# ruizhecao96/CMGAN

Measured on AMD Instinct MI355X. Metric: enhanced audio frames/sec (16 kHz, 2 s clips, batch 32 per GPU), higher is better.
Workload: dtype f32 storage/accumulate; products as 3 x f16 split MFMA (fp32-class accuracy); 1 GPU; configs[1]: batch=32 x 2 s synthetic 16 kHz noisy clips per GPU, n_fft=400 hop=100, TSCNet(64,201) random-init, full pipeline wav->wav; mfma_mode=f16x3, launch=hipGraph replay, batch_per_gpu=32, global_batch=32, frames_per_clip=321, parallelism=dp1

## Files before the change

### cmgan_amd/csrc/attn32_x3.hip

```cpp
#if defined(X3_SINGLE) && defined(A32_STAMP)
#undef A32_STAMP
#endif
#include "kernels.h"
#include <string.h>
#include <stdlib.h>

namespace X3_NS {

typedef float f32x16 __attribute__((ext_vector_type(16)));

__device__ __forceinline__ f32x16 mfma3216(f16x8 a, f16x8 b, f32x16 c) {
    return __builtin_amdgcn_mfma_f32_32x32x16_f16(a, b, c, 0, 0, 0);
}
__device__ __forceinline__ f32x16 mfma3216l(f16x8 a, f16x8 b, f32x16 c) {
    return X3_TERMS == 3 ? __builtin_amdgcn_mfma_f32_32x32x16_f16(a, b, c, 0, 0, 0) : c;
}
__device__ __forceinline__ f32x16 zero16() {
    f32x16 z;
#pragma unroll
    for (int i = 0; i < 16; ++i) z[i] = 0.f;
    return z;
}
#ifdef A32_STAMP
#define A32_SLOTS 2048
__device__ unsigned long long g_a32_stamp[A32_SLOTS][64];
struct A32Stamp {
    unsigned long long t, acc[16];
    int chunks;
};
#define A32_STAMP_ARG , A32Stamp& sp
#define A32_STAMP_PASS , sp
#define A32_STAMP_PTR , A32Stamp* spp
#define A32_STAMP_PTRPASS , &sp
#define A32_MARK(ph)                                            \
    do {                                                        \
        __builtin_amdgcn_sched_barrier(0);                      \
        const unsigned long long _t = __builtin_readcyclecounter(); \
        sp.acc[ph] += _t - sp.t;                                \
        sp.t = _t;                                              \
        __builtin_amdgcn_sched_barrier(0);                      \
    } while (0)
#else
#define A32_STAMP_ARG
#define A32_STAMP_PASS
#define A32_STAMP_PTR
#define A32_STAMP_PTRPASS
#define A32_MARK(ph) do { } while (0)
#endif

__device__ __forceinline__ float red_h_max(float v) {
    float b;
    const float a = xchg32(v, b);
    return fmaxf(a, b);
}
__device__ __forceinline__ float red_h_sum(float v) {
    float b;
    const float a = xchg32(v, b);
    return a + b;
}

#ifndef XCD_ORDER
#define XCD_ORDER 1
#endif
#define XNTB 2
#define XWAVES 8

__device__ __forceinline__ void ln_split32(const f32x4 (&x)[4], f16x8 (&bh)[2], f16x8 (&bl)[2]) {
    float mean, rstd;
    ln_stats(x, mean, rstd);
    f32x4 xh[4];
#pragma unroll
    for (int kb = 0; kb < 4; ++kb) xh[kb] = (x[kb] - splat4(mean)) * splat4(rstd);
    split8(xh[0], xh[1], bh[0], bl[0]);
    split8(xh[2], xh[3], bh[1], bl[1]);
}

__global__ __launch_bounds__(512) void qkv32_x3_kernel(const float* __restrict__ x, TokMap m, int Lt,
                                                       const _Float16* __restrict__ wi, const float* __restrict__ b,
                                                       _Float16* __restrict__ qimg, _Float16* __restrict__ kimg,
                                                       _Float16* __restrict__ vimg, int ntiles) {
    __shared__ __attribute__((aligned(16))) _Float16 wlds[24576];
    __shared__ float scratch[XWAVES * 32 * 17];
    __shared__ __attribute__((aligned(16))) float bias_l[192];
    stage_lds16<3072, 512>(wi, wlds);
    for (int i = threadIdx.x; i < 192; i += blockDim.x) bias_l[i] = b[i];
    __syncthreads();
    const int lane = threadIdx.x & 63, c = lane & 15, g = lane >> 4, wv = threadIdx.x >> 6;
    const int row32 = lane & 31, hh = lane >> 5;
    float* T = scratch + wv * (32 * 17);

#pragma unroll 1
    for (int tile = blockIdx.x * XWAVES + wv; tile < ntiles; tile += gridDim.x * XWAVES) {
        const int n = tile / Lt, it = tile - n * Lt;
        f16x8 xbh[XNTB][2], xbl[XNTB][2];
#pragma unroll
        for (int tb = 0; tb < XNTB; ++tb) {
            int l = it * 32 + tb * 16 + c;
            if (l >= m.L) l = m.L - 1;
            const long row = (long)(n / m.inner) * m.outer + (long)(n % m.inner) * m.istride + (long)l * m.lstride;
            f32x4 xr[4];
#pragma unroll
            for (int kb = 0; kb < 4; ++kb) xr[kb] = ldg4(x + row * 64 + 16 * kb + 4 * g);
            ln_split32(xr, xbh[tb], xbl[tb]);
        }
#pragma unroll 2
        for (int ob = 0; ob < 12; ++ob) {
            const f32x4 bias = *reinterpret_cast<const f32x4*>(&bias_l[16 * ob + 4 * g]);
            f32x4 acc[XNTB];
#pragma unroll
            for (int tb = 0; tb < XNTB; ++tb) acc[tb] = bias;
            lin_acc_x3<2, XNTB>(wlds + ob * 2048 + lane * 8, xbh, xbl, acc);
            const int which = ob >> 2, h = ob & 3;
            const long nh = (long)n * 4 + h;
            if (which < 2) {
                _Float16* img = (which == 0 ? qimg : kimg) + (nh * Lt + it) * 1024;
#pragma unroll
                for (int tb = 0; tb < XNTB; ++tb) {
                    f16x4 hi, lo;
                    split4(acc[tb], hi, lo);
                    _Float16* p = img + ((g >> 1) * 32 + 16 * tb + c) * 8 + 4 * (g & 1);
                    *reinterpret_cast<f16x4*>(p) = hi;
                    *reinterpret_cast<f16x4*>(p + 512) = lo;
                }
            } else {
                wave_lds_fence();
#pragma unroll
                for (int tb = 0; tb < XNTB; ++tb)
#pragma unroll
                    for (int r = 0; r < 4; ++r) T[(16 * tb + c) * 17 + 4 * g + r] = acc[tb][r];
                wave_lds_fence();
#pragma unroll
                for (int grp = 0; grp < 2; ++grp) {
                    f32x4 va, vb;
#pragma unroll
                    for (int r = 0; r < 4; ++r) {
                        va[r] = T[(16 * grp + 4 * hh + r) * 17 + (row32 & 15)];
                        vb[r] = T[(16 * grp + 8 + 4 * hh + r) * 17 + (row32 & 15)];
                    }
                    f16x8 vh, vl;
                    split8(va, vb, vh, vl);
                    const f16x8 out = row32 < 16 ? vh : vl;
                    *reinterpret_cast<f16x8*>(vimg + ((nh * Lt + it) * 2 + grp) * 512 + lane * 8) = out;
                }
            }
        }
    }
}

#ifndef A32_OCC
#define A32_OCC 2
#endif
#ifndef A32_RSEQ
#define A32_RSEQ 1
#endif
#define A32_HI 12.0f
#define A32_LO -4.0f
#define A32_RFL (96 * 32)

struct A32State {
    float m, run, l;
};

typedef unsigned u32x4v __attribute__((ext_vector_type(4)));
__device__ __forceinline__ __amdgpu_buffer_rsrc_t a32_rsrc(const void* base, unsigned bytes) {
    return __builtin_amdgcn_make_buffer_rsrc(const_cast<void*>(base), 0, bytes, 0x00020000);
}
__device__ __forceinline__ f16x8 buf_h8(__amdgpu_buffer_rsrc_t r, unsigned voff, unsigned soff) {
    return __builtin_bit_cast(f16x8, __builtin_amdgcn_raw_buffer_load_b128(r, voff, soff, 0));
}

struct A32Ctx {
    __amdgpu_buffer_rsrc_t qr, kr, vr, er;
    unsigned lane16, eoff, eplane2;
    float* R;
    int wbase, rbase;
    int Lt, L, max_pos, i0, a, hh;
    const unsigned char* mk;
    const char* xbase;
    const char* bo;
};

__device__ __forceinline__ void a32_load_e(const A32Ctx& c, int i0, int n, int t, f16x8& eh, f16x8& el) {
    int row = c.max_pos - (i0 - 64 * n + 32 - 32 * t) + c.a;
#ifdef A32_FAKEE
    row = c.max_pos - 32 + 32 * t + c.a;
#endif
    row = row < 0 ? 0 : (row > 2 * c.max_pos ? 2 * c.max_pos : row);
    const unsigned off = (unsigned)row * 16u + c.eoff;
    eh = buf_h8(c.er, off, 0);
    el = buf_h8(c.er, off, c.eplane2);
}
__device__ __forceinline__ void a32_load_k(const A32Ctx& c, int n, int jt, f16x8& kh, f16x8& kl) {
    int kt = 2 * n + jt;
    kt = kt < c.Lt ? kt : c.Lt - 1;
#ifdef A32_FAKEKV
    kt = jt;
#endif
    kh = buf_h8(c.kr, c.lane16, (unsigned)kt * 2048u);
    kl = buf_h8(c.kr, c.lane16 + 1024u, (unsigned)kt * 2048u);
}
__device__ __forceinline__ f16x8 a32_load_v(const A32Ctx& c, int n, int grp4) {
    int gr = 4 * n + grp4;
    gr = gr < 2 * c.Lt ? gr : 2 * c.Lt - 1;
#ifdef A32_FAKEKV
    gr = grp4 & 1;
#endif
    return buf_h8(c.vr, c.lane16, (unsigned)gr * 1024u);
}

template <int NKT, bool FULL, bool MASK>
__device__ __forceinline__ void a32_softmax(f32x16 (&s)[2], const A32Ctx& c, int j0, A32State& st, f32x16& o,
                                            bool qvalid A32_STAMP_PTR) {
    float mx = -INFINITY;
#pragma unroll
    for (int jt = 0; jt < NKT; ++jt) {
#pragma unroll
        for (int v = 0; v < 16; ++v) {
            float xv = s[jt][v] - st.m;
            const int key = j0 + 32 * jt + 8 * (v >> 2) + 4 * c.hh + (v & 3);
            if (!FULL) xv = key < c.L ? xv : -INFINITY;
            if (MASK && (FULL || key < c.L)) xv = qvalid ? (c.mk[key] ? xv : -INFINITY) : 0.f;
            s[jt][v] = xv;
            mx = fmaxf(mx, xv);
        }
    }
    const float run = fmaxf(st.run, red_h_max(mx));
#ifdef A32_STAMP
    if (spp) { A32Stamp& sp = *spp; A32_MARK(11); }
#endif
    const bool dead = MASK && run == -INFINITY;
    const bool drift = !dead && (run > A32_HI || run < A32_LO);
    float runk = run;
    if (__any(drift)) {
        const float shift = dead ? 0.f : run;
        const float alpha = st.l > 0.f ? __builtin_amdgcn_exp2f(-shift) : 1.0f;
#pragma unroll
        for (int jt = 0; jt < NKT; ++jt)
#pragma unroll
            for (int v = 0; v < 16; ++v) s[jt][v] -= shift;
        st.l *= alpha;
#pragma unroll
        for (int v = 0; v < 16; ++v) o[v] *= alpha;
        st.m += shift;
        if (!dead) runk = 0.f;
    }
    st.run = runk;
    float psum = 0.f;
#pragma unroll
    for (int jt = 0; jt < NKT; ++jt)
#pragma unroll
        for (int v = 0; v < 16; ++v) {
            const float p = __builtin_amdgcn_exp2f(s[jt][v]);
            s[jt][v] = p;
            psum += p;
        }
    st.l += psum;
}

template <int NKT, bool FULL, bool LAST, bool MASK>
__device__ __forceinline__ void a32_chunk(const A32Ctx& c, int n, int i0n, int nn, f16x8& qh, f16x8& ql, f16x8 (&eh)[3], f16x8 (&el)[3],
                                          f16x8 (&kh)[2], f16x8 (&kl)[2], f16x8 (&va)[4], A32State& st, f32x16& o,
                                          bool qvalid, const unsigned (&xo)[2], f32x4 (&xold)[2], f32x4& bias
                                          A32_STAMP_ARG) {
    constexpr int NT = NKT + 1;
#ifndef A32_NO_R
#pragma unroll
    for (int t = 0; t < NT; ++t) {
        f32x16 r = mfma3216(eh[t], qh, zero16());
        if (t == 0) A32_MARK(8);
        r = mfma3216l(eh[t], ql, r);
        r = mfma3216l(el[t], qh, r);
#pragma unroll
        for (int v = 0; v < 16; ++v) c.R[c.wbase + (32 * t + 8 * (v >> 2) + (v & 3)) * 32] = r[v];
        if (A32_RSEQ && (t & 1)) __builtin_amdgcn_sched_barrier(0);
    }
#ifndef A32_NO_LD
#pragma unroll
    for (int t = 0; t < 3; ++t) a32_load_e(c, i0n, nn, t, eh[t], el[t]);
#endif
#endif
    A32_MARK(1);
    wave_lds_fence();
    f32x16 s[2];
#ifndef A32_NO_R
#pragma unroll
    for (int jt = 0; jt < NKT; ++jt) {
#pragma unroll
        for (int v = 0; v < 16; ++v) s[jt][v] = c.R[c.rbase + (32 * jt + 8 * (v >> 2) + (v & 3)) * 32];
    }
#else
    s[0] = zero16(); s[1] = zero16();
#endif
    wave_lds_fence();
    A32_MARK(9);
#pragma unroll
    for (int jt = 0; jt < NKT; ++jt) {
        s[jt] = mfma3216(kh[jt], qh, s[jt]);
        s[jt] = mfma3216l(kh[jt], ql, s[jt]);
        s[jt] = mfma3216l(kl[jt], qh, s[jt]);
    }
#ifndef A32_NO_LD
#pragma unroll
    for (int jt = 0; jt < 2; ++jt) a32_load_k(c, nn, jt, kh[jt], kl[jt]);
    if (LAST) {
        const int itn = (i0n >> 5) < c.Lt ? (i0n >> 5) : c.Lt - 1;
        qh = buf_h8(c.qr, c.lane16, (unsigned)itn * 2048u);
        ql = buf_h8(c.qr, c.lane16 + 1024u, (unsigned)itn * 2048u);
    }
#endif
    A32_MARK(2);
#ifndef A32_NO_SM
    a32_softmax<NKT, FULL, MASK>(s, c, 64 * n, st, o, qvalid A32_STAMP_PTRPASS);
#else
    st.l += s[0][0] + s[1][5];
#endif
    A32_MARK(3);
    if (LAST) {
#pragma unroll
        for (int i = 0; i < 2; ++i) xold[i] = *reinterpret_cast<const f32x4*>(c.xbase + xo[i]);
        bias = *reinterpret_cast<const f32x4*>(c.bo + (c.lane16 >> 8) * 16u);
    }
#ifdef A32_NO_PV
#pragma unroll
    for (int v = 0; v < 16; ++v) o[v] += s[0][v] + s[1][v];
#else
#pragma unroll
    for (int jt = 0; jt < NKT; ++jt) {
#pragma unroll
        for (int half = 0; half < 2; ++half) {
            f32x4 pa, pb;
#pragma unroll
            for (int r = 0; r < 4; ++r) {
                pa[r] = s[jt][8 * half + r];
                pb[r] = s[jt][8 * half + 4 + r];
            }
            f16x8 ph, pl;
            split8(pa, pb, ph, pl);
            o = mfma3216(va[2 * jt + half], ph, o);
            if (jt == 0 && half == 0) A32_MARK(10);
            o = mfma3216l(va[2 * jt + half], pl, o);
        }
    }
#endif
#ifndef A32_NO_LD
#pragma unroll
    for (int g4 = 0; g4 < 4; ++g4) va[g4] = a32_load_v(c, nn, g4);
#endif
    A32_MARK(4);
#ifdef A32_STAMP
    ++sp.chunks;
#endif
}

#ifndef A32_TPB
#define A32_TPB 4
#endif
#ifndef A32_TPB_SHORT
#define A32_TPB_SHORT 16
#endif
#ifndef A32_SLOTS_PER_GPU
#define A32_SLOTS_PER_GPU 512
#endif
#ifndef A32_PERSIST_LONG
#define A32_PERSIST_LONG 0
#endif
#ifndef A32_GROUP
#define A32_GROUP 64
#endif
template <bool MASK>
__global__ __launch_bounds__(256, MASK ? 1 : A32_OCC) void attn32_out_x3_kernel(const _Float16* __restrict__ qimg,
                                                                     const _Float16* __restrict__ kimg,
                                                                     const _Float16* __restrict__ vimg,
                                                                     const _Float16* __restrict__ eimg, int max_pos,
                                                                     float* __restrict__ x, TokMap m,
                                                                     const _Float16* __restrict__ woi,
                                                                     const float* __restrict__ bo, int Lt, int tpb,
                                                                     int bps, long nblocks,
                                                                     const unsigned char* __restrict__ mask) {
    __shared__ __attribute__((aligned(16))) float rbuf[4][A32_RFL];
    __shared__ __attribute__((aligned(16))) f32x4 stash[2][4][2][64];
    __shared__ __attribute__((aligned(16))) _Float16 wo_l[8192];
#ifdef A32_LONE
    __shared__ float lone_pad[8192];
    if (max_pos < 0) lone_pad[threadIdx.x] = 1.f;
#endif
#ifdef A32_STAMP
    A32Stamp sp;
    sp.t = __builtin_readcyclecounter();
    sp.chunks = 0;
#pragma unroll
    for (int i = 0; i < 16; ++i) sp.acc[i] = 0;
#endif
    const int lane = threadIdx.x & 63, wv = __builtin_amdgcn_readfirstlane(threadIdx.x >> 6);
    const long lblk = XCD_ORDER ? (long)(blockIdx.x & 7) * (gridDim.x >> 3) + (blockIdx.x >> 3) : (long)blockIdx.x;
    if (lblk >= nblocks) return;
    stage_lds16<1024, 256>(woi, wo_l);
    const int n = __builtin_amdgcn_readfirstlane((int)((unsigned)lblk / (unsigned)bps));
    const int it0 = ((int)lblk - n * bps) * tpb, it1 = it0 + tpb < Lt ? it0 + tpb : Lt;
    const long nh = (long)n * 4 + wv;
    const int L = m.L;
    A32Ctx c;
    c.a = lane & 31; c.hh = lane >> 5;
    c.R = rbuf[wv];
    c.wbase = 4 * c.hh * 32 + c.a;
    c.rbase = (32 + 4 * c.hh - c.a) * 32 + c.a;
    c.Lt = Lt; c.L = L; c.max_pos = max_pos;
    c.kr = a32_rsrc(kimg + nh * Lt * 1024, (unsigned)Lt * 2048u);
    c.vr = a32_rsrc(vimg + nh * Lt * 1024, (unsigned)Lt * 2048u);
    c.er = a32_rsrc(eimg, (unsigned)(2 * max_pos + 1) * 64u);
    c.qr = a32_rsrc(qimg + nh * Lt * 1024, (unsigned)Lt * 2048u);
    c.lane16 = (unsigned)lane * 16u;
    c.eoff = (unsigned)c.hh * (unsigned)(2 * max_pos + 1) * 16u;
    c.eplane2 = (unsigned)(2 * max_pos + 1) * 32u;
    c.mk = MASK ? mask + (long)n * L : nullptr;
    const int c16 = lane & 15, g16 = lane >> 4;
    const int nq = __builtin_amdgcn_readfirstlane(n / m.inner);
    char* xbase = reinterpret_cast<char*>(x + ((long)nq * m.outer + (long)(n - nq * m.inner) * m.istride) * 64 + 16 * wv);
    const unsigned xstride = (unsigned)m.lstride * 256u, xlane = (unsigned)g16 * 16u;

    c.xbase = xbase;
    c.bo = reinterpret_cast<const char*>(bo + 16 * wv);
    f16x8 qh = buf_h8(c.qr, c.lane16, (unsigned)it0 * 2048u), ql = buf_h8(c.qr, c.lane16 + 1024u, (unsigned)it0 * 2048u);
    f16x8 eh[3], el[3], kh[2], kl[2], va[4];
#pragma unroll
    for (int t = 0; t < 3; ++t) a32_load_e(c, 32 * it0, 0, t, eh[t], el[t]);
#pragma unroll
    for (int jt = 0; jt < 2; ++jt) a32_load_k(c, 0, jt, kh[jt], kl[jt]);
#pragma unroll
    for (int g4 = 0; g4 < 4; ++g4) va[g4] = a32_load_v(c, 0, g4);
    const int nfull = L >> 6, tail = L & 63;
    A32_MARK(0);

#pragma unroll 1
    for (int it = it0; it < it1; ++it) {
        c.i0 = 32 * it;
        bool qvalid = true;
        if (MASK) {
            const int lq = c.i0 + c.a;
            qvalid = c.mk[lq < L ? lq : L - 1] != 0;
        }
        A32State st;
        st.m = 0.f; st.run = -INFINITY; st.l = 0.f;
        f32x16 o = zero16();
        const int i0x = c.i0 + 32;
        unsigned xo[2];
        f32x4 xold[2], bias;
#pragma unroll
        for (int i = 0; i < 2; ++i) {
            const int l = c.i0 + 16 * i + c16;
            xo[i] = (unsigned)(l < L ? l : L - 1) * xstride + xlane;
        }
#define A32_ARGS qh, ql, eh, el, kh, kl, va, st, o, qvalid, xo, xold, bias A32_STAMP_PASS
        if (tail) {
#pragma unroll 1
            for (int ch = 0; ch < nfull; ++ch) a32_chunk<2, true, false, MASK>(c, ch, c.i0, ch + 1, A32_ARGS);
            if (tail > 32) a32_chunk<2, false, true, MASK>(c, nfull, i0x, 0, A32_ARGS);
            else a32_chunk<1, false, true, MASK>(c, nfull, i0x, 0, A32_ARGS);
        } else {
#pragma unroll 1
            for (int ch = 0; ch + 1 < nfull; ++ch) a32_chunk<2, true, false, MASK>(c, ch, c.i0, ch + 1, A32_ARGS);
            a32_chunk<2, true, true, MASK>(c, nfull - 1, i0x, 0, A32_ARGS);
        }
#undef A32_ARGS
        const float inv = __builtin_amdgcn_rcpf(red_h_sum(st.l));
        f32x4 oa, ob;
#pragma unroll
        for (int r = 0; r < 4; ++r) {
            oa[r] = (o[r] + o[8 + r]) * inv;
            ob[r] = (o[4 + r] + o[12 + r]) * inv;
        }
#ifdef A32_NO_EPI
        if (c.i0 + c16 < L) *reinterpret_cast<f32x4*>(xbase + xo[0]) = oa + ob + xold[0] + xold[1] + bias;
        continue;
#endif
        const int par = (it - it0) & 1;
        const _Float16* wp = wo_l + wv * 2048 + lane * 8;
        stash[par][wv][c.a >> 4][c.hh * 16 + (c.a & 15)] = oa;
        stash[par][wv][c.a >> 4][(2 + c.hh) * 16 + (c.a & 15)] = ob;
        A32_MARK(5);
#ifndef A32_NO_BAR
        __syncthreads();
#endif
        A32_MARK(6);
        const f16x8 ah0 = *reinterpret_cast<const f16x8*>(wp), al0 = *reinterpret_cast<const f16x8*>(wp + 512);
        const f16x8 ah1 = *reinterpret_cast<const f16x8*>(wp + 1024), al1 = *reinterpret_cast<const f16x8*>(wp + 1536);
#pragma unroll
        for (int i = 0; i < 2; ++i) {
            f16x8 bh0, bl0, bh1, bl1;
            split8(stash[par][0][i][lane], stash[par][1][i][lane], bh0, bl0);
            split8(stash[par][2][i][lane], stash[par][3][i][lane], bh1, bl1);
            f32x4 acc = bias;
            acc = mfma32h(ah0, bh0, acc);
            acc = mfma32l(ah0, bl0, acc);
            acc = mfma32l(al0, bh0, acc);
            acc = mfma32h(ah1, bh1, acc);
            acc = mfma32l(ah1, bl1, acc);
            acc = mfma32l(al1, bh1, acc);
            if (c.i0 + 16 * i + c16 < L) *reinterpret_cast<f32x4*>(xbase + xo[i]) = xold[i] + acc;
        }
        A32_MARK(7);
    }
#ifdef A32_STAMP
    if (lane == 0) {
        const int b = L < 200 ? 32 : 0;
        unsigned long long* slot = g_a32_stamp[(blockIdx.x * 4 + (threadIdx.x >> 6)) & (A32_SLOTS - 1)];
#pragma unroll
        for (int i = 0; i < 16; ++i) atomicAdd(&slot[b + i], sp.acc[i]);
        atomicAdd(&slot[b + 16], 1ull);
        atomicAdd(&slot[b + 17], (unsigned long long)sp.chunks);
    }
#endif
}

#ifdef A32_STAMP
extern "C" int cmgan_dbg_a32_stamps(unsigned long long* out, int reset) {
    hipDeviceSynchronize();
    static unsigned long long host[A32_SLOTS][64];
    hipError_t e = hipMemcpyFromSymbol(host, HIP_SYMBOL(g_a32_stamp), sizeof host);
    for (int i = 0; i < 64; ++i) {
        out[i] = 0;
        for (int sl = 0; sl < A32_SLOTS; ++sl) out[i] += host[sl][i];
    }
    if (e == hipSuccess && reset) {
        memset(host, 0, sizeof host);
        e = hipMemcpyToSymbol(HIP_SYMBOL(g_a32_stamp), host, sizeof host);
    }
    return e == hipSuccess ? 0 : -1;
}
#endif

#ifndef ASP_OCC
#define ASP_OCC 2
#endif
#define ASP_P 100
#define ASP_RFL (32 * ASP_P)
#define ASP_SB() __builtin_amdgcn_sched_barrier(0)
#if defined(A32_STAMP) && (A32_STAMP + 0 == 2)
#define ASP_FMARK(ph) do { } while (0)
#define ASP_CMARK(ph) A32_MARK(ph)
#else
#define ASP_FMARK(ph) A32_MARK(ph)
#define ASP_CMARK(ph) do { } while (0)
#endif
#ifndef ASP_ABL
#define ASP_ABL 0
#endif

__device__ __forceinline__ f32x16 splat16(float v) {
    f32x16 z;
#pragma unroll
    for (int i = 0; i < 16; ++i) z[i] = v;
    return z;
}

struct AspCtx {
    __amdgpu_buffer_rsrc_t qr, kr, vr, er;
    unsigned lane16, evoff, eplane2;
    float* Rw;
    const float* Rr;
    int Lt, L, max_pos, a, hh, lpad;
};

template <bool CLAMP>
__device__ __forceinline__ void asp_load_e(const AspCtx& c, int i0, int n, int t, f16x8& eh, f16x8& el) {
    if (CLAMP) {
        int row = c.max_pos - (i0 - 64 * n + 32 - 32 * t) + c.a;
        row = row < 0 ? 0 : (row > 2 * c.max_pos ? 2 * c.max_pos : row);
        const unsigned off = (unsigned)row * 16u + c.evoff;
        eh = buf_h8(c.er, off, 0);
        el = buf_h8(c.er, off, c.eplane2);
    } else {
        i0 = i0 < c.lpad ? i0 : c.lpad;
        const unsigned so = (unsigned)(64 * n + 32 * t - i0 + c.lpad) * 16u;
        eh = buf_h8(c.er, c.evoff, so);
        el = buf_h8(c.er, c.evoff, so + c.eplane2);
    }
}
__device__ __forceinline__ void asp_load_k(const AspCtx& c, unsigned so, int n, int jt, f16x8& kh, f16x8& kl) {
    int kt = 2 * n + jt;
    kt = kt < c.Lt ? kt : c.Lt - 1;
    kh = buf_h8(c.kr, c.lane16, so + (unsigned)kt * 2048u);
    kl = buf_h8(c.kr, c.lane16 + 1024u, so + (unsigned)kt * 2048u);
}
__device__ __forceinline__ f16x8 asp_load_v(const AspCtx& c, unsigned so, int n, int grp4) {
    int gr = 4 * n + grp4;
    gr = gr < 2 * c.Lt ? gr : 2 * c.Lt - 1;
    return buf_h8(c.vr, c.lane16, so + (unsigned)gr * 1024u);
}
__device__ __forceinline__ void asp_load_q(const AspCtx& c, unsigned so, int it, f16x8& qh, f16x8& ql) {
    it = it < c.Lt ? it : c.Lt - 1;
    qh = buf_h8(c.qr, c.lane16, so + (unsigned)it * 2048u);
    ql = buf_h8(c.qr, c.lane16 + 1024u, so + (unsigned)it * 2048u);
}
struct AspTile {
    unsigned so;
    int it;
};

__device__ __forceinline__ f32x16 asp_eq(const f16x8& eh, const f16x8& el, const f16x8& qh, const f16x8& ql,
                                         const f32x16& negm) {
    f32x16 r = mfma3216(eh, qh, negm);
    r = mfma3216l(eh, ql, r);
    return mfma3216l(el, qh, r);
}
__device__ __forceinline__ void asp_wwrite(const AspCtx& c, int t, const f32x16& r) {
#pragma unroll
    for (int k = 0; k < 4; ++k) {
        f32x4 w = {r[4 * k], r[4 * k + 1], r[4 * k + 2], r[4 * k + 3]};
        *reinterpret_cast<f32x4*>(c.Rw + 32 * t + 8 * k) = w;
    }
}
template <int NKT>
__device__ __forceinline__ void asp_wread(const AspCtx& c, f32x16 (&sn)[2]) {
#pragma unroll
    for (int jt = 0; jt < NKT; ++jt)
#pragma unroll
        for (int v = 0; v < 16; ++v) sn[jt][v] = c.Rr[32 * jt + 8 * (v >> 2) + (v & 3)];
}
__host__ __device__ constexpr int asp_koff(int jt, int v) { return 32 * jt + 8 * (v >> 2) + (v & 3); }
template <int TAILK = 0>
__device__ __forceinline__ void asp_exp8(const f32x16 (&s)[2], int g, float& psum, f16x8& ph, f16x8& pl) {
    if (ASP_ABL == 3) {
        f32x4 a = {s[g >> 1][8 * (g & 1)], s[g >> 1][8 * (g & 1) + 1], s[g >> 1][8 * (g & 1) + 2], s[g >> 1][8 * (g & 1) + 3]};
        f32x4 b = {s[g >> 1][8 * (g & 1) + 4], s[g >> 1][8 * (g & 1) + 5], s[g >> 1][8 * (g & 1) + 6], s[g >> 1][8 * (g & 1) + 7]};
        ph = __builtin_bit_cast(f16x8, a); pl = __builtin_bit_cast(f16x8, b);
        psum += a[0];
        return;
    }
    f32x4 pa, pb;
#pragma unroll
    for (int r = 0; r < 4; ++r) {
        const bool la = TAILK == 0 || asp_koff(g >> 1, 8 * (g & 1) + r) < TAILK;
        const bool lb = TAILK == 0 || asp_koff(g >> 1, 8 * (g & 1) + 4 + r) < TAILK;
        pa[r] = la ? __builtin_amdgcn_exp2f(s[g >> 1][8 * (g & 1) + r]) : 0.f;
        pb[r] = lb ? __builtin_amdgcn_exp2f(s[g >> 1][8 * (g & 1) + 4 + r]) : 0.f;
        if (la) psum += pa[r];
        if (lb) psum += pb[r];
    }
    asm volatile("" : "+v"(psum));
    split8(pa, pb, ph, pl);
}
__host__ __device__ constexpr int asp_live_groups(int TAILK, int NKT) { return TAILK > 0 ? (TAILK + 15) / 16 : 2 * NKT; }
__device__ __forceinline__ void asp_pv(f32x16& o, const f16x8& va, const f16x8& ph, const f16x8& pl) {
    if (ASP_ABL == 4 || ASP_ABL == 10) {
        o[0] += (float)ph[0] + (float)pl[0] + (float)va[0];
        return;
    }
    o = mfma3216(va, ph, o);
    o = mfma3216l(va, pl, o);
}

template <int NKT, bool CLAMP, bool LASTQ>
__device__ __forceinline__ void asp_front(const AspCtx& c, AspTile tn, int nn, f16x8& qh, f16x8& ql,
                                          f16x8 (&eh)[3], f16x8 (&el)[3], f16x8 (&kh)[2], f16x8 (&kl)[2],
                                          const f32x16& negm, f32x16 (&sn)[2]) {
#pragma unroll
    for (int t = 0; t <= NKT; ++t) {
        const f32x16 r = asp_eq(eh[t], el[t], qh, ql, negm);
        asp_wwrite(c, t, r);
        ASP_SB();
    }
    if (!LASTQ) { eh[0] = eh[2]; el[0] = el[2]; }
#pragma unroll
    for (int t = LASTQ ? 0 : 1; t < 3; ++t) asp_load_e<CLAMP>(c, 32 * tn.it, nn, t, eh[t], el[t]);
    wave_lds_fence();
    asp_wread<NKT>(c, sn);
    wave_lds_fence();
#pragma unroll
    for (int jt = 0; jt < NKT; ++jt) sn[jt] = asp_eq(kh[jt], kl[jt], qh, ql, sn[jt]);
    if (LASTQ) asp_load_q(c, tn.so, tn.it, qh, ql);
#pragma unroll
    for (int jt = 0; jt < 2; ++jt) asp_load_k(c, tn.so, nn, jt, kh[jt], kl[jt]);
    if (LASTQ) __builtin_amdgcn_s_waitcnt(0x0f70);
}

template <int NKT, int TAILK = 0>
__device__ __forceinline__ void asp_back(f32x16 (&s)[2], A32State& st, f32x16& o, const f16x8 (&va)[4]) {
    float psum = 0.f;
#pragma unroll
    for (int g = 0; g < asp_live_groups(TAILK, NKT); ++g) {
        f16x8 ph, pl;
        asp_exp8<TAILK>(s, g, psum, ph, pl);
        asp_pv(o, va[g], ph, pl);
    }
    st.l += psum;
}

template <int NKT, bool FULL, int TAILK = 0>
__device__ __forceinline__ float asp_max(const AspCtx& c, f32x16 (&s)[2], int j0) {
    float mx[2] = {-INFINITY, -INFINITY};
#pragma unroll
    for (int jt = 0; jt < NKT; ++jt)
#pragma unroll
        for (int v = 0; v < 16; ++v) {
            if (!FULL && TAILK > 0) {
                const int koff = asp_koff(jt, v);
                if (koff >= TAILK) { s[jt][v] = -INFINITY; continue; }
                if (koff + 4 >= TAILK) s[jt][v] = c.hh ? -INFINITY : s[jt][v];
            } else if (!FULL) {
                const int key = j0 + 32 * jt + 8 * (v >> 2) + 4 * c.hh + (v & 3);
                s[jt][v] = key < c.L ? s[jt][v] : -INFINITY;
            }
            mx[jt] = fmaxf(mx[jt], s[jt][v]);
        }
    return red_h_max(fmaxf(mx[0], mx[1]));
}

template <int NKT, bool FULL, int TAILK = 0>
__device__ __forceinline__ void asp_reference(const AspCtx& c, f32x16 (&s)[2], int j0, A32State& st, f32x16& o,
                                              f32x16& negm) {
    const float run = fmaxf(st.run, asp_max<NKT, FULL, TAILK>(c, s, j0));
    const bool drift = run > A32_HI || run < A32_LO;
    if (__builtin_expect(__any(drift), 0)) {
        asm volatile("; re-reference");
        const float alpha = st.l > 0.f ? __builtin_amdgcn_exp2f(-run) : 1.0f;
#pragma unroll
        for (int jt = 0; jt < NKT; ++jt)
#pragma unroll
            for (int v = 0; v < 16; ++v) s[jt][v] -= run;
        st.l *= alpha;
#pragma unroll
        for (int v = 0; v < 16; ++v) o[v] *= alpha;
        st.m += run;
        negm = splat16(-st.m);
        st.run = 0.f;
    } else {
        st.run = run;
    }
}

template <int NF, int NB, bool HOTMX, bool CLAMP, bool LASTQ, bool ESHARE = false, int TB = 0>
__device__ __forceinline__ float asp_fused(const AspCtx& c, AspTile tn, int nn, AspTile tv, int vn, f16x8& qh,
                                           f16x8& ql, f16x8 (&eh)[3], f16x8 (&el)[3], f16x8 (&kh)[2], f16x8 (&kl)[2],
                                           f16x8 (&va)[4], const f32x16& negm_n, f32x16 (&s)[2], f32x16 (&sn)[2],
                                           A32State& st, f32x16& o A32_STAMP_ARG) {
    constexpr int LG = asp_live_groups(TB, NB);
    float psum = 0.f;
    f16x8 ph[2], pl[2];
    f32x16 racc = zero16();
    asm volatile("" : "+v"(s[0]), "+v"(s[1]));
    {
        f32x16 r;
        if (ASP_ABL != 2 && ASP_ABL != 10) r = asp_eq(eh[0], el[0], qh, ql, negm_n);
        if (!ESHARE && ASP_ABL != 1 && ASP_ABL != 6 && ASP_ABL != 10) asp_load_e<CLAMP>(c, 32 * tn.it, nn, 0, eh[0], el[0]);
        asp_exp8<TB>(s, 0, psum, ph[0], pl[0]);
        if (ASP_ABL == 8) racc = r; else if (ASP_ABL != 2 && ASP_ABL != 10) asp_wwrite(c, 0, r);
    }
    ASP_FMARK(1);
    ASP_SB();
    {
        f32x16 r;
        if (ASP_ABL != 2 && ASP_ABL != 10) r = asp_eq(eh[1], el[1], qh, ql, negm_n);
        if (ASP_ABL != 1 && ASP_ABL != 6 && ASP_ABL != 10) asp_load_e<CLAMP>(c, 32 * tn.it, nn, 1, eh[1], el[1]);
        asp_pv(o, va[0], ph[0], pl[0]);
        if (ASP_ABL != 1 && ASP_ABL != 7 && ASP_ABL != 10) va[0] = asp_load_v(c, tv.so, vn, 0);
        if (LG > 1) asp_exp8<TB>(s, 1, psum, ph[1], pl[1]);
        if (ASP_ABL == 8) { for (int v = 0; v < 16; ++v) racc[v] = fmaxf(racc[v], r[v]); } else if (ASP_ABL != 2 && ASP_ABL != 10) asp_wwrite(c, 1, r);
    }
    ASP_FMARK(2);
    ASP_SB();
    {
        f32x16 r;
        if (NF == 2 && ASP_ABL != 2 && ASP_ABL != 10) r = asp_eq(eh[2], el[2], qh, ql, negm_n);
        if (ESHARE) { eh[0] = eh[2]; el[0] = el[2]; }
        if (ASP_ABL != 1 && ASP_ABL != 6 && ASP_ABL != 10) asp_load_e<CLAMP>(c, 32 * tn.it, nn, 2, eh[2], el[2]);
        if (LG > 1) asp_pv(o, va[1], ph[1], pl[1]);
        if (ASP_ABL != 1 && ASP_ABL != 7 && ASP_ABL != 10) va[1] = asp_load_v(c, tv.so, vn, 1);
        if (LG > 2) asp_exp8<TB>(s, 2, psum, ph[0], pl[0]);
        if (ASP_ABL == 8) sn[1] = r; else if (NF == 2 && ASP_ABL != 2 && ASP_ABL != 10) asp_wwrite(c, 2, r);
    }
    ASP_FMARK(3);
    ASP_SB();
    wave_lds_fence();
    if (ASP_ABL == 8) sn[0] = racc;
    else if (ASP_ABL != 2 && ASP_ABL != 10) asp_wread<NF>(c, sn);
    else { sn[0] = splat16(psum); sn[1] = splat16(psum); }
    wave_lds_fence();
    if (LG > 2) asp_pv(o, va[2], ph[0], pl[0]);
    if (ASP_ABL != 1 && ASP_ABL != 7 && ASP_ABL != 10) va[2] = asp_load_v(c, tv.so, vn, 2);
    if (LG > 3) asp_exp8<TB>(s, 3, psum, ph[1], pl[1]);
    ASP_FMARK(4);
    ASP_SB();
#pragma unroll
    for (int jt = 0; jt < NF; ++jt)
        if (ASP_ABL != 5 && ASP_ABL != 10) sn[jt] = asp_eq(kh[jt], kl[jt], qh, ql, sn[jt]);
    if (LASTQ) asp_load_q(c, tn.so, tn.it, qh, ql);
    if (ASP_ABL != 1 && ASP_ABL != 7 && ASP_ABL != 10) {
#pragma unroll
        for (int jt = 0; jt < 2; ++jt) asp_load_k(c, tn.so, nn, jt, kh[jt], kl[jt]);
    }
    ASP_FMARK(5);
    ASP_SB();
    if (LG > 3) asp_pv(o, va[3], ph[1], pl[1]);
    if (ASP_ABL != 1 && ASP_ABL != 7 && ASP_ABL != 10) va[3] = asp_load_v(c, tv.so, vn, 3);
    st.l += psum;
    float mx = 0.f;
    if (HOTMX && ASP_ABL != 9) mx = asp_max<2, true>(c, sn, 0);
    ASP_FMARK(6);
#ifdef A32_STAMP
    ++sp.chunks;
#endif
    return mx;
}

template <bool CLAMP, int NKTL, bool FULLL, int TAILK = 0>
__global__ __launch_bounds__(256, ASP_OCC) void attn_sp_out_x3_kernel(const _Float16* __restrict__ qimg,
                                                                const _Float16* __restrict__ kimg,
                                                                const _Float16* __restrict__ vimg,
                                                                const _Float16* __restrict__ eimg, int max_pos,
                                                                float* __restrict__ x, TokMap m,
                                                                const _Float16* __restrict__ woi,
                                                                const float* __restrict__ bo, int Lt, int tpb, int nseq,
                                                                int group, unsigned lt_magic) {
    __shared__ __attribute__((aligned(16))) float rbuf[4][ASP_RFL];
    __shared__ __attribute__((aligned(16))) f32x4 stash[2][4][2][64];
#ifdef A32_STAMP
    A32Stamp sp;
    sp.t = __builtin_readcyclecounter();
    sp.chunks = 0;
#pragma unroll
    for (int i = 0; i < 16; ++i) sp.acc[i] = 0;
#endif
    const int lane = threadIdx.x & 63, wv = __builtin_amdgcn_readfirstlane(threadIdx.x >> 6);
    const int xcd = XCD_ORDER ? (int)(blockIdx.x & 7) : 0, li = XCD_ORDER ? (int)(blockIdx.x >> 3) : (int)blockIdx.x;
    const int nbx = XCD_ORDER ? (int)(gridDim.x >> 3) : (int)gridDim.x;
    const int grp = li / group, gleft = nbx - grp * group;
    const int gs = gleft < group ? gleft : group;
    const int GN = nseq * Lt;
    const int G0 = (xcd * nbx + grp * group) * tpb + (li - grp * group);
    if (G0 >= GN) return;
    const int nleft = (GN - 1 - G0) / gs + 1;
    const int ntl = nleft < tpb ? nleft : tpb;
    auto div_lt = [&](int G) -> int {
        if (__builtin_expect(lt_magic == 0u, 0)) {
            asm volatile("; division path");
            return __builtin_amdgcn_readfirstlane((int)((unsigned)G / (unsigned)Lt));
        }
        return (int)__umulhi((unsigned)__builtin_amdgcn_readfirstlane(G), lt_magic);
    };
    const int n0 = div_lt(G0);
    const long nh0 = (long)n0 * 4 + wv;
    const int L = m.L;
    AspCtx c;
    c.a = lane & 31; c.hh = lane >> 5;
    c.Rw = rbuf[wv] + c.a * ASP_P + 4 * c.hh;
    c.Rr = rbuf[wv] + c.a * (ASP_P - 1) + 32 + 4 * c.hh;
    c.Lt = Lt; c.L = L; c.max_pos = max_pos; c.lpad = 32 * Lt;
    const unsigned long left = ((unsigned long)nseq * 4 - (unsigned long)nh0) * Lt * 2048ul;
    const unsigned span = left < 0xffffffc0ul ? (unsigned)left : 0xffffffc0u;
    c.kr = a32_rsrc(kimg + nh0 * Lt * 1024, span);
    c.vr = a32_rsrc(vimg + nh0 * Lt * 1024, span);
    c.qr = a32_rsrc(qimg + nh0 * Lt * 1024, span);
    c.er = a32_rsrc(eimg, (unsigned)(2 * max_pos + 1) * 64u);
    c.lane16 = (unsigned)lane * 16u;
    c.eplane2 = (unsigned)(2 * max_pos + 1) * 32u;
    c.evoff = (unsigned)c.hh * (unsigned)(2 * max_pos + 1) * 16u;
    if (!CLAMP) c.evoff += (unsigned)(max_pos - 32 + c.a - c.lpad) * 16u;
    const int c16 = lane & 15, g16 = lane >> 4;
    const unsigned seq_bytes = (unsigned)Lt * 8192u;
    const unsigned xstride = (unsigned)m.lstride * 256u, xlane = (unsigned)g16 * 16u;
    const _Float16* wp = woi + wv * 2048 + lane * 8;
    auto tile_of = [&](int G) -> AspTile {
        G = G < GN ? G : GN - 1;
        const int n = div_lt(G);
        AspTile t;
        t.it = G - n * Lt;
        t.so = (unsigned)(n - n0) * seq_bytes;
        return t;
    };

    f16x8 qh, ql, eh[3], el[3], kh[2], kl[2], va[4];
    {
        const AspTile t0 = tile_of(G0);
        asp_load_q(c, t0.so, t0.it, qh, ql);
#pragma unroll
        for (int t = 0; t < 3; ++t) asp_load_e<CLAMP>(c, 32 * t0.it, 0, t, eh[t], el[t]);
#pragma unroll
        for (int jt = 0; jt < 2; ++jt) asp_load_k(c, t0.so, 0, jt, kh[jt], kl[jt]);
#pragma unroll
        for (int g4 = 0; g4 < 4; ++g4) va[g4] = asp_load_v(c, t0.so, 0, g4);
    }
    const int nfull = L >> 6, tail = L & 63;
    const int nch = nfull + (tail ? 1 : 0);

    A32State st;
    st.m = 0.f; st.run = -INFINITY; st.l = 0.f;
    f32x16 o = zero16(), negm = zero16();
    f32x16 s[2];
    if (nch == 1) asp_front<NKTL, CLAMP, true>(c, tile_of(G0 + gs), 0, qh, ql, eh, el, kh, kl, negm, s);
    else asp_front<2, CLAMP, false>(c, tile_of(G0), 1, qh, ql, eh, el, kh, kl, negm, s);

    ASP_CMARK(0);
#pragma unroll 1
    for (int tl = 0; tl < ntl; ++tl) {
        const int G = G0 + tl * gs;
        const AspTile tc = tile_of(G), t1 = tile_of(G + gs);
        const int i0 = 32 * tc.it;
        const int n = n0 + (int)(tc.so / seq_bytes);
        const int nq = __builtin_amdgcn_readfirstlane(n / m.inner);
        char* xbase = reinterpret_cast<char*>(x + ((long)nq * m.outer + (long)(n - nq * m.inner) * m.istride) * 64 + 16 * wv);
        if (nch > 1) asp_reference<2, true>(c, s, 0, st, o, negm);
        else asp_reference<NKTL, FULLL, TAILK>(c, s, 0, st, o, negm);
        int ch = 0;
        while (ch < nch - 2) {
            bool drifted, odd = false;
            f32x16 sn[2];
            do {
                ASP_FMARK(0);
                float mx = asp_fused<2, 2, true, CLAMP, false, true>(c, tc, ch + 2, tc, ch + 1, qh, ql, eh, el, kh, kl, va, negm, s, sn,
                                                               st, o A32_STAMP_PASS);
                st.run = fmaxf(st.run, mx);
                drifted = __any(st.run > A32_HI || st.run < A32_LO);
                ++ch;
                if (!(ch < nch - 2) || drifted) { odd = true; break; }
                ASP_FMARK(0);
                mx = asp_fused<2, 2, true, CLAMP, false, true>(c, tc, ch + 2, tc, ch + 1, qh, ql, eh, el, kh, kl, va, negm, sn, s, st,
                                                         o A32_STAMP_PASS);
                st.run = fmaxf(st.run, mx);
                drifted = __any(st.run > A32_HI || st.run < A32_LO);
                ++ch;
            } while (ch < nch - 2 && !drifted);
            if (odd) { s[0] = sn[0]; s[1] = sn[1]; }
            if (drifted) asp_reference<2, true>(c, s, 0, st, o, negm);
        }
        if (ch < nch - 1) {
            f32x16 sn[2];
            asp_fused<NKTL, 2, false, CLAMP, true>(c, t1, 0, tc, nch - 1, qh, ql, eh, el, kh, kl, va, negm, s, sn,
                                                   st, o A32_STAMP_PASS);
            asp_reference<NKTL, FULLL, TAILK>(c, sn, 64 * nfull, st, o, negm);
            s[0] = sn[0]; s[1] = sn[1];
        }
        unsigned xo[2];
        f32x4 xold[2], bias;
#pragma unroll
        for (int i = 0; i < 2; ++i) {
            const int l = i0 + 16 * i + c16;
            xo[i] = (unsigned)(l < L ? l : L - 1) * xstride + xlane;
            if (!CLAMP) xold[i] = *reinterpret_cast<const f32x4*>(xbase + xo[i]);
        }
        if (!CLAMP) bias = ldg4(bo + 16 * wv + 4 * g16);
        f32x16 sn[2];
        if (tl + 1 < ntl) {
            const f32x16 zero = zero16();
            if (nch == 1) asp_fused<NKTL, NKTL, false, CLAMP, true, false, TAILK>(c, tile_of(G + 2 * gs), 0, t1, 0, qh, ql, eh, el, kh, kl, va, zero, s, sn, st, o A32_STAMP_PASS);
            else asp_fused<2, NKTL, false, CLAMP, false, true, TAILK>(c, t1, 1, t1, 0, qh, ql, eh, el, kh, kl, va, zero, s, sn, st, o A32_STAMP_PASS);
        } else {
            asp_back<NKTL, TAILK>(s, st, o, va);
        }
        ASP_CMARK(1);
        if (CLAMP) {
#pragma unroll
            for (int i = 0; i < 2; ++i) xold[i] = *reinterpret_cast<const f32x4*>(xbase + xo[i]);
            bias = ldg4(bo + 16 * wv + 4 * g16);
        }
        const f16x8 ah0 = *reinterpret_cast<const f16x8*>(wp), al0 = *reinterpret_cast<const f16x8*>(wp + 512);
        const f16x8 ah1 = *reinterpret_cast<const f16x8*>(wp + 1024), al1 = *reinterpret_cast<const f16x8*>(wp + 1536);
        const float inv = __builtin_amdgcn_rcpf(red_h_sum(st.l));
        f32x4 oa, ob;
#pragma unroll
        for (int r = 0; r < 4; ++r) {
            oa[r] = (o[r] + o[8 + r]) * inv;
            ob[r] = (o[4 + r] + o[12 + r]) * inv;
        }
        const int par = tl & 1;
        stash[par][wv][c.a >> 4][c.hh * 16 + (c.a & 15)] = oa;
        stash[par][wv][c.a >> 4][(2 + c.hh) * 16 + (c.a & 15)] = ob;
        st.m = 0.f; st.run = -INFINITY; st.l = 0.f;
        o = zero16(); negm = zero16();
        s[0] = sn[0]; s[1] = sn[1];
        if (ASP_ABL == 11) {
            if (i0 + c16 < L) asm volatile("global_store_dwordx4 %0, %1, %2\n\ts_nop 1" ::"v"(xo[0]), "v"(oa + ob + xold[0] + bias), "s"(xbase) : "memory");
            continue;
        }
        ASP_CMARK(2);
        __syncthreads();
        ASP_CMARK(3);
#pragma unroll
        for (int i = 0; i < 2; ++i) {
            f16x8 bh0, bl0, bh1, bl1;
            split8(stash[par][0][i][lane], stash[par][1][i][lane], bh0, bl0);
            split8(stash[par][2][i][lane], stash[par][3][i][lane], bh1, bl1);
            f32x4 acc = bias;
            acc = mfma32h(ah0, bh0, acc);
            acc = mfma32l(ah0, bl0, acc);
            acc = mfma32l(al0, bh0, acc);
            acc = mfma32h(ah1, bh1, acc);
            acc = mfma32l(ah1, bl1, acc);
            acc = mfma32l(al1, bh1, acc);
            const f32x4 xnew = xold[i] + acc;
            if (i0 + 16 * i + c16 < L)
                asm volatile("global_store_dwordx4 %0, %1, %2\n\ts_nop 1" ::"v"(xo[i]), "v"(xnew), "s"(xbase) : "memory");
        }
        ASP_CMARK(4);
    }
#ifdef A32_STAMP
    ASP_FMARK(0);
    if (lane == 0) {
        const int b = L < 200 ? 32 : 0;
        unsigned long long* slot = g_a32_stamp[(blockIdx.x * 4 + (threadIdx.x >> 6)) & (A32_SLOTS - 1)];
#pragma unroll
        for (int i = 0; i < 16; ++i) atomicAdd(&slot[b + i], sp.acc[i]);
        atomicAdd(&slot[b + 16], 1ull);
        atomicAdd(&slot[b + 17], (unsigned long long)sp.chunks);
    }
#endif
}

}
using namespace X3_NS;

void launch_qkv32_x3(LaunchCtx ctx, const float* x, const TokMap& seq, const _Float16* wi, const float* b,
                     _Float16* qimg, _Float16* kimg, _Float16* vimg) {
    const int N = seq.nblocks / seq.Lb, Lt = (seq.L + 31) / 32;
    const int ntiles = N * Lt;
    const int want = (ntiles + XWAVES - 1) / XWAVES;
    const int grid = want < 512 ? (want > 0 ? want : 1) : 512;
    LAUNCH(ctx, "qkv", (qkv32_x3_kernel<<<grid, 512, 0, ctx.stream>>>(x, seq, Lt, wi, b, qimg, kimg, vimg, ntiles)));
}

void launch_attn32_out_x3(LaunchCtx ctx, const _Float16* qimg, const _Float16* kimg, const _Float16* vimg,
                          const _Float16* rel_img, int max_pos, float* x, const TokMap& seq, const _Float16* woi,
                          const float* bo, const unsigned char* mask) {
    const int N = seq.nblocks / seq.Lb, Lt = (seq.L + 31) / 32;
    const int bps = (Lt + A32_TPB - 1) / A32_TPB;
    const int tpb = (Lt + bps - 1) / bps;
    const long nb = (long)N * bps;
    const unsigned grid = XCD_ORDER ? (unsigned)(((nb + 7) / 8) * 8) : (unsigned)nb;
    LAUNCH(ctx, "attn_out", (attn32_out_x3_kernel<true><<<grid, 256, 0, ctx.stream>>>(
                                qimg, kimg, vimg, rel_img, max_pos, x, seq, woi, bo, Lt, tpb, bps, nb, mask)));
}

#ifndef A32_GROUP_SHORT
#define A32_GROUP_SHORT A32_GROUP
#endif
#ifndef A32_ALIGN_SHORT
#define A32_ALIGN_SHORT 0
#endif
void launch_attn_sp_out_x3(LaunchCtx ctx, const _Float16* qimg, const _Float16* kimg, const _Float16* vimg,
                           const _Float16* rel_img, int max_pos, float* x, const TokMap& seq, const _Float16* woi,
                           const float* bo) {
    const int N = seq.nblocks / seq.Lb, Lt = (seq.L + 31) / 32;
    static const int k_tpb_long = env_knob("CMGAN_ASP_TPB_LONG", A32_TPB, 1, 64), k_group_long = env_knob("CMGAN_ASP_GROUP_LONG", A32_GROUP, 1, 4096);
    static const int k_group_short = env_knob("CMGAN_ASP_GROUP_SHORT", A32_GROUP_SHORT, 1, 4096);
    static const int k_align_short = env_knob("CMGAN_ASP_ALIGN_SHORT", A32_ALIGN_SHORT, 0, 1);
    static const int k_slots = env_knob("CMGAN_ASP_SLOTS", A32_SLOTS_PER_GPU, 8, 65536);
    int tpb = Lt <= 4 ? A32_TPB_SHORT : k_tpb_long;
    if (Lt <= 4 || A32_PERSIST_LONG) {
        const long share = ((long)N * Lt + k_slots - 1) / k_slots;
        if (share > tpb) tpb = (int)share;
        if (Lt <= 4 && k_align_short) tpb = (tpb + Lt - 1) / Lt * Lt;
    }
    const int group = Lt <= 4 ? k_group_short : k_group_long;
    const unsigned lt_magic = Lt > 1 && (long)N * Lt * Lt < (1l << 32) ? (unsigned)((1ul << 32) / (unsigned long)Lt) + 1u : 0u;
    const long nb = ((long)N * Lt + tpb - 1) / tpb;
    const unsigned grid = XCD_ORDER ? (unsigned)(((nb + 7) / 8) * 8) : (unsigned)nb;
    const int tail = seq.L & 63;
    const bool clamp = seq.L + 96 > max_pos;
#define ASP_LAUNCH(CL, NK, FU, ...)                                                                               \
    LAUNCH(ctx, "attn_out", (attn_sp_out_x3_kernel<CL, NK, FU, ##__VA_ARGS__><<<grid, 256, 0, ctx.stream>>>(      \
                                qimg, kimg, vimg, rel_img, max_pos, x, seq, woi, bo, Lt, tpb, N, group, lt_magic)))
    if (!clamp) {
        static const int k_tailk = env_knob("CMGAN_ASP_TAILK", 1, 0, 1);
        if (tail == 0) ASP_LAUNCH(false, 2, true);
        else if (k_tailk && tail == 1) ASP_LAUNCH(false, 1, false, 1);
        else if (k_tailk && tail == 37) ASP_LAUNCH(false, 2, false, 37);
        else if (k_tailk && tail == 45) ASP_LAUNCH(false, 2, false, 45);
        else if (tail > 32) ASP_LAUNCH(false, 2, false);
        else ASP_LAUNCH(false, 1, false);
    } else {
        if (tail == 0) ASP_LAUNCH(true, 2, true);
        else if (tail > 32) ASP_LAUNCH(true, 2, false);
        else ASP_LAUNCH(true, 1, false);
    }
#undef ASP_LAUNCH
}
```

Baseline: 484,700 frames/s.

## Handle single stray key separately so tail-1 attention runs full-chunk path

When the sequence length leaves exactly one key beyond a multiple of 64 (e.g. L=321), the kernel now treats the last key as a stray. Its score is computed with scalar FMAs and used to seed the softmax state, and its V row seeds the accumulator. The remaining L-1 keys then run through the full-chunk MFMA path instead of an extra tail chunk. This avoids a whole mostly-empty 64-key chunk of MFMA work per tile, at the cost of extra scalar loads and per-lane reductions and some risk to softmax state correctness.

```diff
diff --git a/cmgan_amd/csrc/attn32_x3.hip b/cmgan_amd/csrc/attn32_x3.hip
--- a/cmgan_amd/csrc/attn32_x3.hip
+++ b/cmgan_amd/csrc/attn32_x3.hip
@@ -803,7 +803,51 @@
     return mx;
 }
 
-template <bool CLAMP, int NKTL, bool FULLL, int TAILK = 0>
+struct AspStray {
+    f16x8 kh, kl, eh, el;
+    _Float16 v[16];
+};
+__device__ __forceinline__ _Float16 buf_h1(__amdgpu_buffer_rsrc_t r, unsigned voff, unsigned soff) {
+    return __builtin_bit_cast(_Float16, __builtin_amdgcn_raw_buffer_load_b16(r, voff, soff, 0));
+}
+__device__ __forceinline__ void asp_load_stray(const AspCtx& c, unsigned sevoff, AspTile t, AspStray& y) {
+    const unsigned ks = t.so + (unsigned)(c.Lt - 1) * 2048u;
+    y.kh = buf_h8(c.kr, (unsigned)c.hh * 512u, ks);
+    y.kl = buf_h8(c.kr, (unsigned)c.hh * 512u, ks + 1024u);
+    const unsigned es = (unsigned)(c.L - 1 - 32 * t.it) * 16u;
+    y.eh = buf_h8(c.er, sevoff, es);
+    y.el = buf_h8(c.er, sevoff, es + c.eplane2);
+    const unsigned vs = t.so + (unsigned)(c.Lt - 1) * 2048u;
+#pragma unroll
+    for (int v = 0; v < 8; ++v) {
+        const unsigned vo = vs + (unsigned)((v >> 2) * 128 + (v & 3) * 16);
+        y.v[v] = buf_h1(c.vr, (unsigned)c.hh * 64u, vo);
+        y.v[8 + v] = buf_h1(c.vr, (unsigned)c.hh * 64u, vo + 256u);
+    }
+}
+__device__ __forceinline__ void asp_stray_init(const AspStray& y, const f16x8& qh, const f16x8& ql, f32x16 (&s)[2],
+                                               A32State& st, f32x16& o, f32x16& negm) {
+    float acc[4] = {0.f, 0.f, 0.f, 0.f};
+#pragma unroll
+    for (int j = 0; j < 8; ++j) {
+        const float q = (float)qh[j] + (float)ql[j];
+        acc[0] = fmaf(q, (float)y.kh[j], acc[0]);
+        acc[1] = fmaf(q, (float)y.kl[j], acc[1]);
+        acc[2] = fmaf(q, (float)y.eh[j], acc[2]);
+        acc[3] = fmaf(q, (float)y.el[j], acc[3]);
+    }
+    const float sx = red_h_sum((acc[0] + acc[2]) + (acc[1] + acc[3]));
+#pragma unroll
+    for (int jt = 0; jt < 2; ++jt)
+#pragma unroll
+        for (int v = 0; v < 16; ++v) s[jt][v] -= sx;
+    st.m = sx; st.run = 0.f; st.l = 0.5f;
+    negm = splat16(-sx);
+#pragma unroll
+    for (int v = 0; v < 16; ++v) o[v] = (float)y.v[v];
+}
+
+template <bool CLAMP, int NKTL, bool FULLL, int TAILK = 0, bool STRAY = false>
 __global__ __launch_bounds__(256, ASP_OCC) void attn_sp_out_x3_kernel(const _Float16* __restrict__ qimg,
                                                                 const _Float16* __restrict__ kimg,
                                                                 const _Float16* __restrict__ vimg,
@@ -856,6 +900,7 @@
     c.eplane2 = (unsigned)(2 * max_pos + 1) * 32u;
     c.evoff = (unsigned)c.hh * (unsigned)(2 * max_pos + 1) * 16u;
     if (!CLAMP) c.evoff += (unsigned)(max_pos - 32 + c.a - c.lpad) * 16u;
+    const unsigned sevoff = (unsigned)c.hh * (unsigned)(2 * max_pos + 1) * 16u + (unsigned)(max_pos - c.a) * 16u;
     const int c16 = lane & 15, g16 = lane >> 4;
     const unsigned seq_bytes = (unsigned)Lt * 8192u;
     const unsigned xstride = (unsigned)m.lstride * 256u, xlane = (unsigned)g16 * 16u;
@@ -880,7 +925,10 @@
 #pragma unroll
         for (int g4 = 0; g4 < 4; ++g4) va[g4] = asp_load_v(c, t0.so, 0, g4);
     }
-    const int nfull = L >> 6, tail = L & 63;
+    AspStray sy;
+    if (STRAY) asp_load_stray(c, sevoff, tile_of(G0), sy);
+    const int Lk = STRAY ? L - 1 : L;
+    const int nfull = Lk >> 6, tail = Lk & 63;
     const int nch = nfull + (tail ? 1 : 0);
 
     A32State st;
@@ -899,6 +947,7 @@
         const int n = n0 + (int)(tc.so / seq_bytes);
         const int nq = __builtin_amdgcn_readfirstlane(n / m.inner);
         char* xbase = reinterpret_cast<char*>(x + ((long)nq * m.outer + (long)(n - nq * m.inner) * m.istride) * 64 + 16 * wv);
+        if (STRAY) asp_stray_init(sy, qh, ql, s, st, o, negm);
         if (nch > 1) asp_reference<2, true>(c, s, 0, st, o, negm);
         else asp_reference<NKTL, FULLL, TAILK>(c, s, 0, st, o, negm);
         int ch = 0;
@@ -955,6 +1004,7 @@
         }
         const f16x8 ah0 = *reinterpret_cast<const f16x8*>(wp), al0 = *reinterpret_cast<const f16x8*>(wp + 512);
         const f16x8 ah1 = *reinterpret_cast<const f16x8*>(wp + 1024), al1 = *reinterpret_cast<const f16x8*>(wp + 1536);
+        if (STRAY) asp_load_stray(c, sevoff, t1, sy);
         const float inv = __builtin_amdgcn_rcpf(red_h_sum(st.l));
         f32x4 oa, ob;
 #pragma unroll
@@ -1061,7 +1111,9 @@
                                 qimg, kimg, vimg, rel_img, max_pos, x, seq, woi, bo, Lt, tpb, N, group, lt_magic)))
     if (!clamp) {
         static const int k_tailk = env_knob("CMGAN_ASP_TAILK", 1, 0, 1);
+        static const int k_stray = env_knob("CMGAN_ASP_STRAY", 1, 0, 1);
         if (tail == 0) ASP_LAUNCH(false, 2, true);
+        else if (k_stray && tail == 1 && seq.L >= 129) ASP_LAUNCH(false, 2, true, 0, true);
         else if (k_tailk && tail == 1) ASP_LAUNCH(false, 1, false, 1);
         else if (k_tailk && tail == 37) ASP_LAUNCH(false, 2, false, 37);
         else if (k_tailk && tail == 45) ASP_LAUNCH(false, 2, false, 45);
```

New measurement: 486,800 frames/s (median of 4 runs). About the same (+0.4%).
